# dotnetpower/infomesh

Hardware: AMD Instinct MI355X
Metric: queries/sec (hybrid BM25+dense search, 1.25M docs) (higher is better)
Workload: dtype bf16; 1 GPU; model=bge-small-en(random-init) encoder + BM25 CSR + cosine top-k, global_batch=128, seq_len=32, parallelism=shard1, mode=hybrid, docs_per_gpu=1250000, total_docs=1250000

## Files before the change

### infomesh_amd/index/gpu_index.py

```python
from __future__ import annotations

import math
import re
from dataclasses import dataclass

import numpy as np
import torch

from ..hashing import hash64
from .doc_attrs import (DEAD_BIT, TOP_FETCH, U32_MAX, DocFilter, FacetSpec,
                        TermOps, domain_tables_np, domain_top_np,
                        facet_counts_np, pack_facets, pack_pred,
                        pack_pred_sets, passes, words_i32)

BM25_K1 = 1.2
BM25_B = 0.75
BM25_VOCAB = 1 << 17

MAX_SEGMENTS = 16

COLLAPSE_M_MAX = 4
COLLAPSE_WS_BYTES = 256 << 20


def per_domain_caps(per_domain, B: int) -> list[int] | None:
# ... 80 lines not shown

    def __init__(self, device: str = "cuda", vocab: int = BM25_VOCAB,
                 emb_dtype: str = "bf16"):
        assert emb_dtype in ("bf16", "fp8")
        self.device = torch.device(device)
        self.vocab = vocab
        self.emb_dtype = emb_dtype
        self.n_docs = 0
        self.segments: list[PostingSegment] = []
        self.df: np.ndarray = np.zeros(vocab, dtype=np.int64)
        self._doc_lens = np.zeros(0, dtype=np.int64)
        self.avgdl = 1.0
        self._emb_buf: torch.Tensor | None = None
        self._gid_buf: torch.Tensor | None = None
        self._attr_buf: torch.Tensor | None = None
        self.n_dead = 0
        self._live_bits = None
        self._dom_tables = None
        self._dom_ws: torch.Tensor | None = None
        self._collapse_ws: dict[str, torch.Tensor] = {}
        self._topk = None
        self._topk_dense = None
        self._topk_pruned = None
        self._dense_bmax: dict = {}
        self._dense_graphs: dict = {}
        self.graph_dense = False
        self._h_idf: np.ndarray | None = None
        self._pend_tokens: list[np.ndarray] = []
        self._pend_emb: list[torch.Tensor] = []
        self._pend_gids: list[int] = []
        self._pend_attrs: list = []

    @property
    def embeddings(self) -> torch.Tensor | None:
        if self._emb_buf is None or self.n_docs == 0:
            return None
        return self._emb_buf[:self.n_docs]

    @property
    def global_ids(self) -> torch.Tensor | None:
        if self._gid_buf is None:
            return None
        return self._gid_buf[:self.n_docs]

    @property
    def attrs(self) -> torch.Tensor | None:
        if self._attr_buf is None:
# ... 231 lines not shown
        dl = dl_dev[docs_u.long()].to(torch.int32)
        tfdl = (tf | (dl << 16)).contiguous()
        df_dev = torch.bincount(terms_u, minlength=self.vocab)
        offsets_dev = torch.zeros(self.vocab + 1, dtype=torch.int64,
                                  device=dev)
        torch.cumsum(df_dev, 0, out=offsets_dev[1:])
        df_new = df_dev.cpu().numpy().astype(np.int64)
        seg = PostingSegment(
            offsets=offsets_dev, doc_ids=docs_u.contiguous(),
            tfdl=tfdl, doc_base=self.n_docs, n_docs=n_new,
            h_offs=offsets_dev.cpu().numpy())
        return seg, df_new

    def _upload_t(self, t: torch.Tensor, stream) -> torch.Tensor:
        pinned = t.contiguous().pin_memory()
        with torch.cuda.stream(stream):
            return pinned.to(self.device, non_blocking=True)

    def _invalidate_query_caches(self) -> None:
        self._h_idf = None
        self._dense_graphs = {}
        self._dense_bufs = {}
        self._dense_bmax = {}
        self._bm25_hists = {}
        self._live_bits = None
        self._dom_tables = None
        self._dom_ws = None

    def optimize(self) -> None:
        if len(self.segments) <= 1:
            return
        dev = self.device
        V = self.vocab
        term_parts, doc_parts, tfdl_parts = [], [], []
        arangeV = torch.arange(V, dtype=torch.int64, device=dev)
        for seg in self.segments:
            dfg = seg.offsets.diff()
            term_parts.append(torch.repeat_interleave(arangeV, dfg))
            doc_parts.append(seg.doc_ids.to(torch.int64) + seg.doc_base)
            tfdl_parts.append(seg.tfdl)
        terms = torch.cat(term_parts)
        docs = torch.cat(doc_parts)
        tfdl = torch.cat(tfdl_parts)
        key = terms * self.n_docs + docs
        key, order = torch.sort(key)
        docs_sorted = (key % self.n_docs).to(torch.int32)
# ... 332 lines not shown
        if mark is None:
            def mark(name, t0):
                return t0
        B = len(queries_terms)
        caps = per_domain_caps(per_domain, B)
        dev = self.device
        N = self.n_docs
        k = min(k, N)
        topk = self._get_topk()
        mask = _mask if _mask is not None else self._mask_for(filters, B,
                                                              term_ops)
        tp = _time.perf_counter()
        if scores_buf is not None and scores_buf.shape == (B, N):
            scores = scores_buf
        else:
            scores = torch.empty(B, N, device=dev, dtype=torch.float32)
        qrows, terms = self.dedupe_terms(queries_terms)
        uterms, qt_ut = np.unique(terms, return_inverse=True)
        idf = self._idf_table()[terms]
        qt_off = np.zeros(B + 1, dtype=np.int64)
        np.cumsum(np.bincount(qrows, minlength=B), out=qt_off[1:])
        bd = self._pick_bd(B)
        U = len(uterms)
        hists = getattr(self, "_bm25_hists", None)
        if hists is None:
            hists = self._bm25_hists = {}
        hist = hists.get(B)
        if hist is None:
            hist = hists[B] = torch.zeros(
                B * 256, device=dev, dtype=torch.int32)
        else:
            hist.zero_()
        tp = mark("shard.chunks", tp)
        evt = getattr(self, "_h2d_evt", None)
        if evt is not None:
            evt.synchronize()
        qt_off_d = self._h2d("qt_off", qt_off, torch.int32)
        qt_ut_d = self._h2d("qt_ut", qt_ut, torch.int32)
        qt_idf_d = self._h2d("qt_idf", idf, torch.float32)
        for si, seg in enumerate(self.segments):
            nblocks = (seg.n_docs + bd - 1) // bd
            bounds = self._bounds_ws(U * nblocks * 2)
            K.bm25_block(
                seg.doc_ids, seg.tfdl, qt_off_d, qt_ut_d, qt_idf_d,
                self._h2d(f"qb{si}", seg.h_offs[uterms], torch.int64),
                self._h2d(f"qe{si}", seg.h_offs[uterms + 1], torch.int64),
                bounds, scores, seg.doc_base, seg.n_docs, bd,
                self.avgdl, k1=BM25_K1, b=BM25_B,
                hist1=hist if mask is None else None)
        if dev.type == "cuda":
            if evt is None:
                evt = self._h2d_evt = torch.cuda.Event()
            evt.record()
        tp = mark("shard.bm25", tp)
        counts = None
        if facets is not None:
            rows_t, edges_t, langs_t, desc_t, doms_t = (
                torch.from_numpy(t) for t in facets.tables())
            counts = K.facet_counts(
                scores, rows_t, self.attrs, edges_t, langs_t, desc_t,
                doms_t, **_mask_kw(mask))
            tp = mark("shard.facets", tp)
        dom_top = tally = None
        if facets is not None and facets.top_rows:
            dom_keys, dom_id = self._domain_tables()
            top_rows = torch.tensor(facets.top_rows, dtype=torch.int32)
            D = dom_keys.numel()
            cnt = K.domain_count(
                scores, top_rows, dom_id, D,
                out=self._domain_ws(len(facets.top_rows), D),
                **_mask_kw(mask))
            dom_top = K.domain_select(cnt, dom_keys, TOP_FETCH + 1)
            tally = DomainTally(cnt, dom_keys)
            tp = mark("shard.topdomains", tp)
        if mask is None:
            out = topk(scores, k, ext_hist1=hist)
        else:
            out = topk(scores, k, mask=mask[0], row_pred=mask[1])
        tp = mark("shard.bm25topk", tp)
        if caps is not None:
            self._collapse_rows("bm25", scores, k, caps, mask, out[0],
                                out[1])
            mark("shard.bm25collapse", tp)
        self._bm25_scores_buf = scores
        return out[0], out[1], counts, dom_top, tally

    def search(self, queries_terms: list[np.ndarray],
               query_emb: torch.Tensor | None, k: int = 100,
               scores_buf: torch.Tensor | None = None,
               phase_t: dict | None = None,
               filters: list[DocFilter | None] | None = None,
               term_ops: list[TermOps | None] | None = None,
               facets: FacetSpec | None = None,
               per_domain: list[int | None] | None = None) -> ShardHits:
        import time as _time

        def mark(name, t0):
            if phase_t is None:
# ... 293 lines not shown
```

### infomesh_amd/ops/_ext.py

```python
from __future__ import annotations

import ctypes
from ctypes import c_float, c_int, c_long, c_void_p
from pathlib import Path

from ..errors import GpuExtensionMissing

_LIB: ctypes.CDLL | None = None
_LOAD_ERROR: str | None = None

_SIGNATURES: dict[str, list] = {
    "infomesh_gemm_bf16_nt": [c_void_p, c_void_p, c_void_p, c_void_p,
                              c_int, c_int, c_int, c_int,
                              c_long, c_long, c_long,
                              c_int, c_float, c_int, c_void_p],
    "infomesh_layernorm": [c_void_p, c_void_p, c_void_p, c_void_p,
                           c_void_p, c_void_p, c_long, c_int, c_float,
                           c_long, c_void_p],
    "infomesh_embed_layernorm": [c_void_p, c_void_p, c_void_p, c_void_p,
                                 c_void_p, c_void_p, c_long, c_int, c_int,
                                 c_float, c_void_p],
    "infomesh_rmsnorm": [c_void_p, c_void_p, c_void_p, c_void_p,
                         c_void_p, c_long, c_int, c_float, c_void_p],
    "infomesh_softmax": [c_void_p, c_void_p, c_void_p, c_long, c_int,
# ... 8 lines not shown
    "infomesh_pool": [c_void_p, c_void_p, c_void_p, c_int, c_int, c_int,
                      c_int, c_int, c_void_p],
    "infomesh_argmax": [c_void_p, c_void_p, c_long, c_int, c_void_p],
    "infomesh_topk": [c_void_p, c_void_p, c_void_p, c_void_p, c_int,
                      c_long, c_int, c_void_p, c_void_p],
    "infomesh_topk_masked": [c_void_p, c_void_p, c_void_p, c_void_p, c_int,
                             c_long, c_int, c_void_p, c_void_p, c_long,
                             c_void_p],
    "infomesh_filter_bitmask": [c_void_p, c_void_p, c_void_p, c_long,
                                c_int, c_void_p],
    "infomesh_filter_bitmask_sets": [c_void_p, c_void_p, c_void_p, c_void_p,
                                     c_void_p, c_long, c_int, c_void_p],
    "infomesh_term_bitmask": [c_void_p, c_long, c_void_p, c_void_p,
                              c_void_p, c_void_p, c_int, c_void_p, c_int,
                              c_long, c_long, c_long, c_long, c_void_p],
    "infomesh_term_block_docs": [],
    "infomesh_topk_workspace_u32": [c_int],
    "infomesh_topk_zero_u32": [c_int],
    "infomesh_bm25_block": [c_void_p, c_void_p, c_void_p, c_void_p,
                            c_void_p, c_void_p, c_void_p, c_void_p,
                            c_void_p, c_void_p, c_int, c_int, c_long,
                            c_long, c_long, c_int, c_float, c_float,
                            c_float, c_void_p],
    "infomesh_score_combine": [c_void_p, c_void_p, c_void_p, c_float,
                               c_float, c_long, c_void_p],
    "infomesh_simhash_fingerprint": [c_void_p, c_void_p, c_void_p, c_long,
                                     c_void_p],
    "infomesh_hamming_scan": [c_void_p, c_void_p, c_void_p, c_void_p,
                              c_void_p, c_void_p, c_int, c_long, c_int,
                              c_int, c_void_p],
    "infomesh_attn_decode": [c_void_p, c_void_p, c_void_p, c_void_p,
                             c_void_p, c_int, c_int, c_int, c_int, c_int,
                             c_float, c_void_p],
    "infomesh_attn_decode_split": [c_void_p, c_void_p, c_void_p, c_void_p,
                                   c_void_p, c_void_p, c_int, c_int, c_int,
                                   c_int, c_int, c_int, c_float, c_void_p],
    "infomesh_attn_fused": [c_void_p, c_void_p, c_void_p, c_void_p,
                            c_void_p, c_int, c_int, c_int, c_int, c_int,
                            c_int, c_long, c_long, c_long, c_long, c_long,
                            c_long, c_long, c_long, c_long,
                            c_long, c_long, c_long,
                            c_int, c_float, c_int, c_void_p],
    "infomesh_kv_append": [c_void_p, c_void_p, c_void_p, c_void_p,
                           c_void_p, c_int, c_int, c_int, c_int, c_void_p],
    "infomesh_dense_scores": [c_void_p, c_void_p, c_void_p,
                              c_int, c_long, c_int, c_float, c_void_p],
# ... 5 lines not shown
                               c_long, c_long, c_long,
                               c_int, c_float, c_int, c_void_p],
    "infomesh_gemv_bf16_nt": [c_void_p, c_void_p, c_void_p, c_void_p,
                              c_int, c_int, c_int, c_int,
                              c_long, c_long, c_long,
                              c_int, c_float, c_int, c_void_p],
    "infomesh_qkv_split": [c_void_p, c_void_p, c_void_p, c_void_p,
                           c_void_p, c_void_p, c_void_p,
                           c_int, c_int, c_int, c_int, c_int, c_int,
                           c_void_p],
    "infomesh_merge_heads": [c_void_p, c_void_p, c_int, c_int, c_int,
                             c_int, c_void_p],
    "infomesh_silu_mul_fused": [c_void_p, c_void_p, c_long, c_int,
                                c_void_p],
    "infomesh_gemm_tile": [c_int, c_int, c_int, c_int],
    "infomesh_gemm_bmax_width": [c_int, c_int, c_int, c_int],
    "infomesh_gemm_bf16_nt_bmax": [c_void_p, c_void_p, c_void_p, c_void_p,
                                   c_void_p, c_int, c_int, c_int, c_int,
                                   c_long, c_long, c_long,
                                   c_int, c_float, c_void_p],
    "infomesh_topk_pruned": [c_void_p, c_void_p, c_int, c_void_p, c_void_p,
                             c_void_p, c_int, c_long, c_int, c_void_p],
    "infomesh_topk_pruned_workspace_u32": [c_int, c_long, c_int, c_int],
    "infomesh_topk_pruned_zero_u32": [c_int],
    "infomesh_facet_counts": [c_void_p, c_void_p, c_void_p, c_void_p,
                              c_void_p, c_void_p, c_void_p, c_void_p,
                              c_void_p, c_long, c_void_p, c_int, c_int,
                              c_long, c_long, c_int, c_int, c_int, c_int,
                              c_void_p],
    "infomesh_facet_chunk_docs": [],
    "infomesh_facet_width": [c_int, c_int, c_int],
    "infomesh_facet_slot": [c_int, c_int, c_int],
    "infomesh_domain_count": [c_void_p, c_void_p, c_void_p, c_void_p,
                              c_void_p, c_void_p, c_int, c_int, c_long,
                              c_long, c_int, c_int, c_void_p],
    "infomesh_domain_select": [c_void_p, c_void_p, c_void_p, c_int, c_int,
                               c_int, c_void_p],
    "infomesh_domtop_chunk_docs": [],
    "infomesh_domtop_lds_slots": [],
    "infomesh_domtop_k_max": [],
    "infomesh_domain_best": [c_void_p, c_void_p, c_void_p, c_void_p,
                             c_void_p, c_void_p, c_int, c_int, c_long,
                             c_long, c_int, c_int, c_int, c_int, c_void_p],
    "infomesh_collapse_select": [c_void_p, c_void_p, c_void_p, c_int, c_int,
                                 c_int, c_int, c_void_p],
    "infomesh_collapse_m_max": [],
    "infomesh_collapse_k_max": [],
    "infomesh_collapse_chunk_docs": [],
    "infomesh_collapse_lds_slots": [],
}

_RESTYPES = {"infomesh_topk_workspace_u32": c_long,
             "infomesh_collapse_m_max": c_int,
             "infomesh_collapse_k_max": c_int,
             "infomesh_collapse_chunk_docs": c_int,
             "infomesh_collapse_lds_slots": c_int,
             "infomesh_domtop_chunk_docs": c_int,
             "infomesh_domtop_lds_slots": c_int,
             "infomesh_domtop_k_max": c_int,
             "infomesh_facet_chunk_docs": c_int,
             "infomesh_facet_width": c_int,
             "infomesh_facet_slot": c_int,
             "infomesh_topk_zero_u32": c_long,
             "infomesh_topk_pruned_workspace_u32": c_long,
             "infomesh_topk_pruned_zero_u32": c_long,
             "infomesh_term_block_docs": c_int,
             "infomesh_gemm_bmax_width": c_int,
             "infomesh_gemm_bf16_nt_bmax": c_int,
             "infomesh_dense_scores": c_int,
             "infomesh_dense_scores_fp8": c_int,
             "infomesh_gemm_tile": c_int,
             "infomesh_attn_fused": c_int,
             "infomesh_embed_layernorm": c_int}


def _try_load() -> ctypes.CDLL | None:
    global _LOAD_ERROR
    so = Path(__file__).resolve().parent / "libinfomesh_hip.so"
    if not so.exists():
        _LOAD_ERROR = f"{so} not built"
        return None
    try:
        lib = ctypes.CDLL(str(so))
    except OSError as e:
        _LOAD_ERROR = str(e)
        return None
    for name, argtypes in _SIGNATURES.items():
        fn = getattr(lib, name)
        fn.argtypes = argtypes
        fn.restype = _RESTYPES.get(name)
    import os
    if os.environ.get("INFOMESH_SYNC_DEBUG"):
        return _SyncDebugLib(lib)
    return lib


class _SyncDebugLib:

    def __init__(self, real: ctypes.CDLL):
        self._real = real

    def __getattr__(self, name: str):
        fn = getattr(self._real, name)
        if not name.startswith("infomesh_"):
            return fn

        def checked(*args, _fn=fn, _name=name):
            r = _fn(*args)
            import torch
            if torch.cuda.is_available():
                try:
                    torch.cuda.synchronize()
                except RuntimeError as e:
# ... 27 lines not shown
```

### infomesh_amd/ops/csrc/bm25.hip

```cpp
#include "common.h"

namespace {

DEVINL long lower_bound_i32(const int* __restrict__ a, long lo, long hi,
                            int v) {
  while (lo < hi) {
    const long mid = (lo + hi) >> 1;
    if (a[mid] < v) lo = mid + 1; else hi = mid;
  }
  return lo;
}

__global__ __launch_bounds__(256) void bm25_bounds_kernel(
    const int* __restrict__ doc_ids,
    const long* __restrict__ u_begin,
    const long* __restrict__ u_end,
    int* __restrict__ bounds,
    int U, int nblocks, int BD) {
  const int i = blockIdx.x * blockDim.x + threadIdx.x;
  if (i >= U * nblocks) return;
  const int ut = i / nblocks, blk = i % nblocks;
  const long b = u_begin[ut], e = u_end[ut];
  const long d0 = (long)blk * BD;
  const long lo = lower_bound_i32(doc_ids, b, e, (int)d0);
  const long hi = lower_bound_i32(doc_ids, lo, e, (int)(d0 + BD));
  bounds[2 * i] = (int)(lo - b);
  bounds[2 * i + 1] = (int)(hi - b);
}

template <bool HIST>
__global__ __launch_bounds__(256) void bm25_block_kernel(
    const int* __restrict__ doc_ids,
    const unsigned int* __restrict__ tfdl,
    const int* __restrict__ qt_off,
    const int* __restrict__ qt_ut,
    const float* __restrict__ qt_idf,
    const long* __restrict__ u_begin,
    const int* __restrict__ bounds,
    float* __restrict__ scores,
    unsigned* __restrict__ hist1,
    long rowN, long doc_base, long nseg, int BD, int nblocks,
    float norm_a, float norm_b, float k1p1) {
  extern __shared__ float lds_scores[];
  const int q = blockIdx.x;
  const int blk = blockIdx.y;
  const long d0 = (long)blk * BD;
  const int nd = (int)min((long)BD, nseg - d0);
  unsigned* lh = reinterpret_cast<unsigned*>(lds_scores + BD);
  for (int i = threadIdx.x; i < nd; i += blockDim.x) lds_scores[i] = 0.0f;
  if (HIST) hist8_zero(lh);
  __syncthreads();
  const int t0 = qt_off[q], t1 = qt_off[q + 1];
  for (int ti = t0; ti < t1; ++ti) {
    const int ut = qt_ut[ti];
    const int* bp = bounds + 2 * ((long)ut * nblocks + blk);
    const long base = u_begin[ut];
    const long lo = base + bp[0], hi = base + bp[1];
    const float w = qt_idf[ti] * k1p1;
    for (long p = lo + threadIdx.x; p < hi; p += blockDim.x) {
      const int d = doc_ids[p] - (int)d0;
      const unsigned int td = tfdl[p];
      const float tf = (float)(td & 0xffffu);
      const float dl = (float)(td >> 16);
      atomicAdd(&lds_scores[d], w * tf / (tf + norm_a + norm_b * dl));
    }
    __syncthreads();
  }
  float* __restrict__ srow = scores + (long)q * rowN + doc_base + d0;
  if (!HIST) {
    for (int i = threadIdx.x; i < nd; i += blockDim.x)
      __builtin_nontemporal_store(lds_scores[i], srow + i);
    return;
  }
  unsigned* my = hist8_mine(lh);
  unsigned zc = 0;
  for (int i = threadIdx.x; i < nd; i += blockDim.x) {
    const float v = lds_scores[i];
    __builtin_nontemporal_store(v, srow + i);
    if (v == 0.0f) ++zc;
    else atomicAdd(&my[float_to_ordered(v) >> 24], 1u);
  }
  for (int off = WAVE / 2; off; off >>= 1)
    zc += __shfl_xor(zc, off, WAVE);
  constexpr unsigned ZBIN = 0x80000000u >> 24;
  if ((threadIdx.x % WAVE) == 0 && zc)
    atomicAdd(&my[ZBIN], zc);
  __syncthreads();
  hist8_merge(lh, hist1 + (long)q * 256);
}

__global__ void combine_kernel(const float* __restrict__ a,
                               const float* __restrict__ b,
                               float* __restrict__ out,
                               float wa, float wb, long n) {
  const long idx = (long)blockIdx.x * blockDim.x + threadIdx.x;
  for (long i = idx; i < n; i += (long)gridDim.x * blockDim.x)
    out[i] = wa * a[i] + wb * b[i];
}

}

extern "C" void infomesh_bm25_block(
    const void* doc_ids, const void* tfdl, const void* qt_off,
    const void* qt_ut, const void* qt_idf, const void* u_begin,
    const void* u_end, void* bounds, void* scores, void* hist1,
    int B, int U, long rowN, long doc_base, long nseg,
    int BD, float norm_a, float norm_b, float k1p1, void* stream) {
  if (nseg <= 0 || B <= 0) return;
  auto s = reinterpret_cast<hipStream_t>(stream);
  const int nblocks = (int)((nseg + BD - 1) / BD);
  if (U > 0) {
    const int total = U * nblocks;
    hipLaunchKernelGGL(bm25_bounds_kernel,
                       dim3((unsigned)((total + 255) / 256)), dim3(256), 0, s,
                       (const int*)doc_ids, (const long*)u_begin,
                       (const long*)u_end, (int*)bounds, U, nblocks, BD);
  }
  dim3 grid((unsigned)B, (unsigned)nblocks);
  const size_t shm = (size_t)BD * sizeof(float)
      + (hist1 ? HIST8_U32 * sizeof(unsigned) : 0);
  if (hist1)
    hipLaunchKernelGGL(bm25_block_kernel<true>, grid, dim3(256), shm, s,
                       (const int*)doc_ids, (const unsigned int*)tfdl,
                       (const int*)qt_off, (const int*)qt_ut,
                       (const float*)qt_idf, (const long*)u_begin,
                       (const int*)bounds, (float*)scores,
                       (unsigned*)hist1,
                       rowN, doc_base, nseg, BD, nblocks,
                       norm_a, norm_b, k1p1);
  else
    hipLaunchKernelGGL(bm25_block_kernel<false>, grid, dim3(256), shm, s,
                       (const int*)doc_ids, (const unsigned int*)tfdl,
                       (const int*)qt_off, (const int*)qt_ut,
                       (const float*)qt_idf, (const long*)u_begin,
                       (const int*)bounds, (float*)scores, nullptr,
                       rowN, doc_base, nseg, BD, nblocks,
                       norm_a, norm_b, k1p1);
}

extern "C" void infomesh_score_combine(const void* a, const void* b,
                                       void* out, float wa, float wb,
                                       long n, void* stream) {
  auto s = reinterpret_cast<hipStream_t>(stream);
  long blocks = min((n + 255) / 256, (long)2048);
  hipLaunchKernelGGL(combine_kernel, dim3((unsigned)blocks), dim3(256), 0, s,
                     (const float*)a, (const float*)b, (float*)out, wa, wb, n);
}
```

### infomesh_amd/ops/csrc/topk.hip

```cpp
#include "common.h"

#define TOPK_CAP 8192

#define HI_RES 4096

namespace {

struct MaskRef {
  const unsigned* bits;
  const int* row_pred;
  long W;
};
DEVINL const unsigned* mask_row(const MaskRef& m, int b) {
  return m.bits + (long)m.row_pred[b] * m.W;
}
DEVINL unsigned mask_nibble(const unsigned* __restrict__ mrow, long i) {
  return (mrow[i >> 3] >> ((unsigned)(i & 7) * 4)) & 15u;
}
DEVINL void keep_loaded(float4& v) {
  asm volatile("" : "+v"(v.x), "+v"(v.y), "+v"(v.z), "+v"(v.w));
}
DEVINL bool mask_bit(const unsigned* __restrict__ mrow, long col) {
  return (mrow[col >> 5] >> (unsigned)(col & 31)) & 1u;
}
// ... 254 lines not shown
      const unsigned long long v = d[i];
      out_vals[(long)b * K + i] = ordered_to_float(~(unsigned)(v >> 32));
      out_idx[(long)b * K + i] = (int)(v & 0xffffffffu);
    } else {
      out_vals[(long)b * K + i] = -INFINITY;
      out_idx[(long)b * K + i] = -1;
    }
  }
}

struct TopkLayout {
  long hist1, hist2, bin1, chi1, thresh, shift, cnt, cnt_eq, cand, total;
  explicit TopkLayout(long B)
      : hist1(0), hist2(hist1 + B * 256), bin1(hist2 + B * 256),
        chi1(bin1 + B), thresh(chi1 + B), shift(thresh + B),
        cnt(shift + B), cnt_eq(cnt + B),
        cand((cnt_eq + B + 1) & ~1L),
        total(cand + B * TOPK_CAP * 2) {}
};
unsigned long long* cand_of(unsigned* ws, long B) {
  return reinterpret_cast<unsigned long long*>(ws + TopkLayout(B).cand);
}

#define PRUNE_THREADS 1024
#define PRUNE_PAD 0xffffffffu
__global__ __launch_bounds__(PRUNE_THREADS) void gather_blocks_kernel(
    const float* __restrict__ scores, const int* __restrict__ ids,
    int* __restrict__ blk, float* __restrict__ gath, long N, long NB,
    int W, int K1) {
  __shared__ int d[1024];
  const int b = blockIdx.x;
  int n2 = 64;
  while (n2 < K1) n2 <<= 1;
  for (int i = threadIdx.x; i < n2; i += blockDim.x)
    d[i] = i < K1 ? ids[(long)b * K1 + i] : 0x7fffffff;
  __syncthreads();
  for (int k = 2; k <= n2; k <<= 1) {
    for (int j = k >> 1; j > 0; j >>= 1) {
      for (int i = threadIdx.x; i < n2; i += blockDim.x) {
        const int ixj = i ^ j;
        if (ixj > i) {
          const bool up = ((i & k) == 0);
          const int a = d[i], c = d[ixj];
          if ((a > c) == up) { d[i] = c; d[ixj] = a; }
        }
      }
      __syncthreads();
    }
  }
  for (int i = threadIdx.x; i < K1; i += blockDim.x)
    blk[(long)b * K1 + i] = d[i];
  const float* row = scores + (long)b * N;
  float* grow = gath + (long)b * K1 * W;
  for (int e = threadIdx.x; e < K1 * W; e += blockDim.x) {
    const long id = d[e / W];
    const long col = id * W + e % W;
    grow[e] = (id >= 0 && id < NB && col < N) ? row[col]
                                              : __uint_as_float(PRUNE_PAD);
  }
}

__global__ __launch_bounds__(256) void remap_blocks_kernel(
    const int* __restrict__ blk, float* __restrict__ out_vals,
    int* __restrict__ out_idx, long N, int W, int K1, int K) {
  const int b = blockIdx.x;
  for (int i = threadIdx.x; i < K; i += blockDim.x) {
    const int p = out_idx[(long)b * K + i];
    if (p < 0) continue;
    const long col = (long)blk[(long)b * K1 + p / W] * W + p % W;
    if (col < N) {
      out_idx[(long)b * K + i] = (int)col;
    } else {
      out_vals[(long)b * K + i] = -INFINITY;
      out_idx[(long)b * K + i] = -1;
    }
  }
}

struct PrunedLayout {
  long K1, zero2, cand, vals1, idx1, blk, gath, total;
  PrunedLayout(long B, long NB, long K, long W)
      : K1(K < NB ? K : NB), zero2(TopkLayout(B).cand), cand(2 * zero2),
        vals1(cand + B * TOPK_CAP * 2), idx1(vals1 + B * K1),
        blk(idx1 + B * K1),
        gath((blk + B * K1 + 3) & ~3L),
        total(gath + B * K1 * W) {}
};

}

extern "C" long infomesh_topk_workspace_u32(int B) {
  return TopkLayout(B).total;
}

extern "C" long infomesh_topk_zero_u32(int B) { return TopkLayout(B).cand; }

template <bool MASKED, typename... M>
static void topk_launch(const void* scores, unsigned* ws,
                        unsigned long long* cand, void* out_vals,
                        void* out_idx, int B, long N, int K,
                        const void* ext_hist1, hipStream_t s, M... mask) {
  static_assert(sizeof...(M) == (MASKED ? 1 : 0), "one MaskRef iff MASKED");
  const TopkLayout L(B);

  int chunks = (int)min((N + 256 * 64 - 1) / (256 * 64), (long)1024);
  if (chunks < 1) chunks = 1;
  dim3 g1(chunks, B), blk(256);
  const unsigned* h1 = (const unsigned*)ext_hist1;
  if (!h1) {
    h1 = ws + L.hist1;
// ... 17 lines not shown
                     (int*)out_idx, K);
}

extern "C" void infomesh_topk(const void* scores, void* workspace,
                              void* out_vals, void* out_idx,
                              int B, long N, int K,
                              const void* ext_hist1, void* stream) {
  unsigned* ws = reinterpret_cast<unsigned*>(workspace);
  topk_launch<false>(scores, ws, cand_of(ws, B), out_vals, out_idx, B, N, K,
                     ext_hist1, reinterpret_cast<hipStream_t>(stream));
}

extern "C" void infomesh_topk_masked(const void* scores, void* workspace,
                                     void* out_vals, void* out_idx,
                                     int B, long N, int K,
                                     const void* bits, const void* row_pred,
                                     long W, void* stream) {
  unsigned* ws = reinterpret_cast<unsigned*>(workspace);
  topk_launch<true>(scores, ws, cand_of(ws, B), out_vals, out_idx, B, N, K,
                    nullptr, reinterpret_cast<hipStream_t>(stream),
                    MaskRef{(const unsigned*)bits, (const int*)row_pred, W});
}

extern "C" long infomesh_topk_pruned_workspace_u32(int B, long N, int K,
                                                   int W) {
  return PrunedLayout(B, (N + W - 1) / W, K, W).total;
}
extern "C" long infomesh_topk_pruned_zero_u32(int B) {
  return 2 * TopkLayout(B).cand;
}

extern "C" void infomesh_topk_pruned(const void* scores, const void* bmax,
                                     int W, void* workspace, void* out_vals,
                                     void* out_idx, int B, long N, int K,
                                     void* stream) {
  hipStream_t s = reinterpret_cast<hipStream_t>(stream);
  unsigned* ws = reinterpret_cast<unsigned*>(workspace);
  const long NB = (N + W - 1) / W;
  const PrunedLayout L(B, NB, K, W);
  const int K1 = (int)L.K1;
  auto* cand = reinterpret_cast<unsigned long long*>(ws + L.cand);
  int* idx1 = reinterpret_cast<int*>(ws + L.idx1);
  int* blk = reinterpret_cast<int*>(ws + L.blk);
  float* gath = reinterpret_cast<float*>(ws + L.gath);
  topk_launch<false>(bmax, ws, cand, ws + L.vals1, idx1, B, NB, K1, nullptr,
                     s);
  hipLaunchKernelGGL(gather_blocks_kernel, dim3(B), dim3(PRUNE_THREADS), 0,
                     s, (const float*)scores, idx1, blk, gath, N, NB, W, K1);
  topk_launch<false>(gath, ws + L.zero2, cand, out_vals, out_idx, B,
                     (long)K1 * W, K, nullptr, s);
  hipLaunchKernelGGL(remap_blocks_kernel, dim3(B), dim3(256), 0, s, blk,
                     (float*)out_vals, (int*)out_idx, N, W, K1, K);
}
```

### infomesh_amd/ops/kernels.py

```python
from __future__ import annotations

import torch

from . import _ext

ACT = {"none": 0, "gelu": 1, "silu": 2, "relu": 3, "tanh": 4}


def _ptr(t: torch.Tensor | None) -> int | None:
    return None if t is None else t.data_ptr()


def _check(t: torch.Tensor, dtype: torch.dtype, name: str) -> None:
    assert t.is_cuda, f"{name} must be on GPU"
    assert t.dtype == dtype, f"{name} must be {dtype}, got {t.dtype}"
    assert t.is_contiguous(), f"{name} must be contiguous"


def gemm_route(M: int, N: int, K: int, G: int) -> str:
    if M <= 16:
        return "gemv"
    if (M >= 4096 and N >= 512 and K % 64 == 0
            and ((M + 255) // 256) * ((N + 255) // 256) * max(G, 1) >= 224):
        return "gemm8"
# ... 312 lines not shown
                scores.data_ptr(), self._ws.data_ptr(), vals.data_ptr(),
                idx.data_ptr(), B, N, k, mask.data_ptr(),
                row_pred.data_ptr(), mask.shape[1], _ext.stream_ptr())
            return vals, idx
        lib.infomesh_topk(scores.data_ptr(), self._ws.data_ptr(),
                          vals.data_ptr(), idx.data_ptr(), B, N, k,
                          0 if ext_hist1 is None else ext_hist1.data_ptr(),
                          _ext.stream_ptr())
        return vals, idx


class TopKPruned:

    def __init__(self, device: torch.device | str = "cuda"):
        self.device = torch.device(device)
        self._ws: torch.Tensor | None = None

    def __call__(self, scores: torch.Tensor, bmax: torch.Tensor, W: int,
                 k: int) -> tuple[torch.Tensor, torch.Tensor]:
        assert scores.dim() == 2
        _check(scores, torch.float32, "scores")
        _check(bmax, torch.float32, "bmax")
        B, N = scores.shape
        assert 1 <= k <= 1024 and W > 0
        assert bmax.shape == (B, (N + W - 1) // W), \
            f"bmax must be [B, ceil(N/W)], got {tuple(bmax.shape)}"
        lib = _ext.lib()
        nu32 = lib.infomesh_topk_pruned_workspace_u32(B, N, k, W)
        if self._ws is None or self._ws.numel() < nu32:
            self._ws = torch.empty(nu32, device=scores.device,
                                   dtype=torch.int32)
        self._ws[:lib.infomesh_topk_pruned_zero_u32(B)].zero_()
        vals = torch.empty((B, k), device=scores.device, dtype=torch.float32)
        idx = torch.empty((B, k), device=scores.device, dtype=torch.int32)
        lib.infomesh_topk_pruned(
            scores.data_ptr(), bmax.data_ptr(), W, self._ws.data_ptr(),
            vals.data_ptr(), idx.data_ptr(), B, N, k, _ext.stream_ptr())
        return vals, idx


def topk(scores: torch.Tensor, k: int) -> tuple[torch.Tensor, torch.Tensor]:
    return TopK(scores.device)(scores, k)


def filter_bitmask(attrs: torch.Tensor, preds: torch.Tensor) -> torch.Tensor:
    _check(attrs, torch.int32, "attrs")
    _check(preds, torch.int32, "preds")
    assert attrs.dim() == 2 and attrs.shape[1] == 4
    assert preds.dim() == 2 and preds.shape[1] == 4 and preds.shape[0] >= 1
    N, P = attrs.shape[0], preds.shape[0]
    assert P <= 65535
    W = (N + 63) // 64 * 2
    bits = torch.empty((P, W), device=attrs.device, dtype=torch.int32)
    _ext.lib().infomesh_filter_bitmask(
        attrs.data_ptr(), preds.data_ptr(), bits.data_ptr(), N, P,
        _ext.stream_ptr())
    return bits


FILTER_SETS_MAX = 2048
# ... 331 lines not shown
    m, R, D = best.shape
    if not 1 <= m <= collapse_m_max():
        raise ValueError(
            f"collapse_select: m = {m}; 1 <= m <= {collapse_m_max()}")
    if not 1 <= k <= collapse_k_max():
        raise ValueError(
            f"collapse_select: k = {k}; 1 <= k <= {collapse_k_max()}")
    assert R >= 1 and D >= 1, "best: [m, R, D]"
    vals = torch.empty((R, k), device=best.device, dtype=torch.float32)
    idx = torch.empty((R, k), device=best.device, dtype=torch.int32)
    _ext.lib().infomesh_collapse_select(
        best.data_ptr(), vals.data_ptr(), idx.data_ptr(), R, D, m, k,
        _ext.stream_ptr())
    return vals, idx


def bm25_block(doc_ids: torch.Tensor, tfdl: torch.Tensor,
               qt_off: torch.Tensor, qt_ut: torch.Tensor,
               qt_idf: torch.Tensor, u_begin: torch.Tensor,
               u_end: torch.Tensor, bounds: torch.Tensor,
               scores: torch.Tensor, doc_base: int, nseg: int,
               bd: int, avgdl: float, k1: float = 1.2,
               b: float = 0.75,
               hist1: torch.Tensor | None = None) -> torch.Tensor:
    B, N = scores.shape
    U = u_begin.numel()
    nblocks = (nseg + bd - 1) // bd
    _check(scores, torch.float32, "scores")
    assert nblocks <= 65535 and qt_off.numel() == B + 1
    assert doc_ids.dtype == torch.int32 and tfdl.dtype == torch.int32
    assert bounds.numel() >= U * nblocks * 2
    assert bd * 4 + (8448 if hist1 is not None else 0) <= 160 * 1024
    if hist1 is not None:
        assert hist1.dtype == torch.int32 and hist1.numel() >= B * 256
    norm_a = k1 * (1.0 - b)
    norm_b = k1 * b / max(avgdl, 1e-9)
    _ext.lib().infomesh_bm25_block(
        doc_ids.data_ptr(), tfdl.data_ptr(), qt_off.data_ptr(),
        qt_ut.data_ptr(), qt_idf.data_ptr(), u_begin.data_ptr(),
        u_end.data_ptr(), bounds.data_ptr(), scores.data_ptr(),
        0 if hist1 is None else hist1.data_ptr(),
        B, U, N, doc_base, nseg, bd,
        norm_a, norm_b, k1 + 1.0, _ext.stream_ptr())
    return scores


def score_combine(a: torch.Tensor, b: torch.Tensor, wa: float,
                  wb: float) -> torch.Tensor:
    out = torch.empty_like(a)
    _ext.lib().infomesh_score_combine(a.data_ptr(), b.data_ptr(),
                                      out.data_ptr(), wa, wb, a.numel(),
                                      _ext.stream_ptr())
    return out


def simhash_fingerprint(offsets: torch.Tensor,
                        hashes: torch.Tensor) -> torch.Tensor:
    ndocs = offsets.numel() - 1
    out = torch.empty(ndocs, device=offsets.device, dtype=torch.int64)
    _ext.lib().infomesh_simhash_fingerprint(
        offsets.data_ptr(), hashes.data_ptr(), out.data_ptr(), ndocs,
        _ext.stream_ptr())
    return out

# ... 129 lines not shown
```

Before: 44570 queries/s.

## Emit per-64-doc block maxima from BM25 and use single-kernel pruned top-k

The BM25 scoring kernel gains a variant that writes, alongside the scores, the maximum score of every 64-document block. The BM25 top-k then goes through a rewritten pruned selector: a row-parallel radix select over block maxima picks candidate blocks, and only those blocks' scores are scanned. This replaces the old multi-launch pruned pipeline (two top-k passes, gather, remap) and the histogram path. The new path is on by default when no filter mask is present, at the cost of an extra bmax buffer and more complex kernels.

```diff
diff --git a/infomesh_amd/index/gpu_index.py b/infomesh_amd/index/gpu_index.py
--- a/infomesh_amd/index/gpu_index.py
+++ b/infomesh_amd/index/gpu_index.py
@@ -1,6 +1,7 @@
 from __future__ import annotations
 
 import math
+import os
 import re
 from dataclasses import dataclass
 
@@ -127,7 +128,10 @@
         self._topk = None
         self._topk_dense = None
         self._topk_pruned = None
+        self._topk_pruned_bm25 = None
         self._dense_bmax: dict = {}
+        self.bm25_pruned = os.environ.get("INFOMESH_BM25_PRUNED") != "0"
+        self._bm25_bmax: dict = {}
         self._dense_graphs: dict = {}
         self.graph_dense = False
         self._h_idf: np.ndarray | None = None
@@ -405,6 +409,7 @@
         self._dense_graphs = {}
         self._dense_bufs = {}
         self._dense_bmax = {}
+        self._bm25_bmax = {}
         self._bm25_hists = {}
         self._live_bits = None
         self._dom_tables = None
@@ -783,15 +788,24 @@
         np.cumsum(np.bincount(qrows, minlength=B), out=qt_off[1:])
         bd = self._pick_bd(B)
         U = len(uterms)
-        hists = getattr(self, "_bm25_hists", None)
-        if hists is None:
-            hists = self._bm25_hists = {}
-        hist = hists.get(B)
-        if hist is None:
-            hist = hists[B] = torch.zeros(
-                B * 256, device=dev, dtype=torch.int32)
-        else:
-            hist.zero_()
+        pruned = (mask is None and self.bm25_pruned and dev.type == "cuda"
+                  and all(s.doc_base % 64 == 0 for s in self.segments))
+        bmax = hist = None
+        if pruned:
+            bmax = self._bm25_bmax.get(B)
+            if bmax is None or bmax.shape != (B, (N + 63) // 64):
+                bmax = self._bm25_bmax[B] = torch.empty(
+                    B, (N + 63) // 64, device=dev, dtype=torch.float32)
+        elif mask is None:
+            hists = getattr(self, "_bm25_hists", None)
+            if hists is None:
+                hists = self._bm25_hists = {}
+            hist = hists.get(B)
+            if hist is None:
+                hist = hists[B] = torch.zeros(
+                    B * 256, device=dev, dtype=torch.int32)
+            else:
+                hist.zero_()
         tp = mark("shard.chunks", tp)
         evt = getattr(self, "_h2d_evt", None)
         if evt is not None:
@@ -808,7 +822,7 @@
                 self._h2d(f"qe{si}", seg.h_offs[uterms + 1], torch.int64),
                 bounds, scores, seg.doc_base, seg.n_docs, bd,
                 self.avgdl, k1=BM25_K1, b=BM25_B,
-                hist1=hist if mask is None else None)
+                hist1=hist, bmax=bmax)
         if dev.type == "cuda":
             if evt is None:
                 evt = self._h2d_evt = torch.cuda.Event()
@@ -834,7 +848,11 @@
             dom_top = K.domain_select(cnt, dom_keys, TOP_FETCH + 1)
             tally = DomainTally(cnt, dom_keys)
             tp = mark("shard.topdomains", tp)
-        if mask is None:
+        if pruned:
+            if self._topk_pruned_bm25 is None:
+                self._topk_pruned_bm25 = K.TopKPruned(dev)
+            out = self._topk_pruned_bm25(scores, bmax, 64, k)
+        elif mask is None:
             out = topk(scores, k, ext_hist1=hist)
         else:
             out = topk(scores, k, mask=mask[0], row_pred=mask[1])
diff --git a/infomesh_amd/ops/_ext.py b/infomesh_amd/ops/_ext.py
--- a/infomesh_amd/ops/_ext.py
+++ b/infomesh_amd/ops/_ext.py
@@ -54,6 +54,11 @@
                             c_void_p, c_void_p, c_int, c_int, c_long,
                             c_long, c_long, c_int, c_float, c_float,
                             c_float, c_void_p],
+    "infomesh_bm25_block_bmax": [c_void_p, c_void_p, c_void_p, c_void_p,
+                                 c_void_p, c_void_p, c_void_p, c_void_p,
+                                 c_void_p, c_void_p, c_int, c_int, c_long,
+                                 c_long, c_long, c_int, c_float, c_float,
+                                 c_float, c_void_p],
     "infomesh_score_combine": [c_void_p, c_void_p, c_void_p, c_float,
                                c_float, c_long, c_void_p],
     "infomesh_simhash_fingerprint": [c_void_p, c_void_p, c_void_p, c_long,
@@ -105,7 +110,6 @@
     "infomesh_topk_pruned": [c_void_p, c_void_p, c_int, c_void_p, c_void_p,
                              c_void_p, c_int, c_long, c_int, c_void_p],
     "infomesh_topk_pruned_workspace_u32": [c_int, c_long, c_int, c_int],
-    "infomesh_topk_pruned_zero_u32": [c_int],
     "infomesh_facet_counts": [c_void_p, c_void_p, c_void_p, c_void_p,
                               c_void_p, c_void_p, c_void_p, c_void_p,
                               c_void_p, c_long, c_void_p, c_int, c_int,
@@ -145,8 +149,8 @@
              "infomesh_facet_width": c_int,
              "infomesh_facet_slot": c_int,
              "infomesh_topk_zero_u32": c_long,
+             "infomesh_topk_pruned": c_int,
              "infomesh_topk_pruned_workspace_u32": c_long,
-             "infomesh_topk_pruned_zero_u32": c_long,
              "infomesh_term_block_docs": c_int,
              "infomesh_gemm_bmax_width": c_int,
              "infomesh_gemm_bf16_nt_bmax": c_int,
@@ -157,6 +161,17 @@
              "infomesh_embed_layernorm": c_int}
 
 
+def bind(so: Path | str, strict: bool = True) -> ctypes.CDLL:
+    lib = ctypes.CDLL(str(so))
+    for name, argtypes in _SIGNATURES.items():
+        if not strict and not hasattr(lib, name):
+            continue
+        fn = getattr(lib, name)
+        fn.argtypes = argtypes
+        fn.restype = _RESTYPES.get(name)
+    return lib
+
+
 def _try_load() -> ctypes.CDLL | None:
     global _LOAD_ERROR
     so = Path(__file__).resolve().parent / "libinfomesh_hip.so"
@@ -164,14 +179,10 @@
         _LOAD_ERROR = f"{so} not built"
         return None
     try:
-        lib = ctypes.CDLL(str(so))
+        lib = bind(so)
     except OSError as e:
         _LOAD_ERROR = str(e)
         return None
-    for name, argtypes in _SIGNATURES.items():
-        fn = getattr(lib, name)
-        fn.argtypes = argtypes
-        fn.restype = _RESTYPES.get(name)
     import os
     if os.environ.get("INFOMESH_SYNC_DEBUG"):
         return _SyncDebugLib(lib)
diff --git a/infomesh_amd/ops/csrc/bm25.hip b/infomesh_amd/ops/csrc/bm25.hip
--- a/infomesh_amd/ops/csrc/bm25.hip
+++ b/infomesh_amd/ops/csrc/bm25.hip
@@ -1,4 +1,5 @@
 #include "common.h"
+#include "gemm_common.h"
 
 namespace {
 
@@ -28,7 +29,7 @@
   bounds[2 * i + 1] = (int)(hi - b);
 }
 
-template <bool HIST>
+template <bool HIST, bool BMAX = false>
 __global__ __launch_bounds__(256) void bm25_block_kernel(
     const int* __restrict__ doc_ids,
     const unsigned int* __restrict__ tfdl,
@@ -39,6 +40,7 @@
     const int* __restrict__ bounds,
     float* __restrict__ scores,
     unsigned* __restrict__ hist1,
+    float* __restrict__ bmax,
     long rowN, long doc_base, long nseg, int BD, int nblocks,
     float norm_a, float norm_b, float k1p1) {
   extern __shared__ float lds_scores[];
@@ -67,6 +69,28 @@
     __syncthreads();
   }
   float* __restrict__ srow = scores + (long)q * rowN + doc_base + d0;
+  if (BMAX) {
+    float* __restrict__ brow =
+        bmax + (long)q * ((rowN + WAVE - 1) / WAVE) + (doc_base + d0) / WAVE;
+    const int lane = threadIdx.x % WAVE;
+    for (int base = 0; base < nd; base += blockDim.x) {
+      const int i = base + threadIdx.x;
+      unsigned bits = 0;
+      if (i < nd) {
+        const float v = lds_scores[i];
+        __builtin_nontemporal_store(v, srow + i);
+        bits = __float_as_uint(v);
+      }
+      bits = group_max_u32<16>(bits);
+      const unsigned m = max(
+          max((unsigned)__builtin_amdgcn_readlane((int)bits, 0),
+              (unsigned)__builtin_amdgcn_readlane((int)bits, 16)),
+          max((unsigned)__builtin_amdgcn_readlane((int)bits, 32),
+              (unsigned)__builtin_amdgcn_readlane((int)bits, 48)));
+      if (lane == 0 && i < nd) brow[i / WAVE] = __uint_as_float(m);
+    }
+    return;
+  }
   if (!HIST) {
     for (int i = threadIdx.x; i < nd; i += blockDim.x)
       __builtin_nontemporal_store(lds_scores[i], srow + i);
@@ -100,11 +124,11 @@
 
 }
 
-extern "C" void infomesh_bm25_block(
+static void bm25_launch(
     const void* doc_ids, const void* tfdl, const void* qt_off,
     const void* qt_ut, const void* qt_idf, const void* u_begin,
     const void* u_end, void* bounds, void* scores, void* hist1,
-    int B, int U, long rowN, long doc_base, long nseg,
+    void* bmax, int B, int U, long rowN, long doc_base, long nseg,
     int BD, float norm_a, float norm_b, float k1p1, void* stream) {
   if (nseg <= 0 || B <= 0) return;
   auto s = reinterpret_cast<hipStream_t>(stream);
@@ -119,13 +143,22 @@
   dim3 grid((unsigned)B, (unsigned)nblocks);
   const size_t shm = (size_t)BD * sizeof(float)
       + (hist1 ? HIST8_U32 * sizeof(unsigned) : 0);
-  if (hist1)
+  if (bmax)
+    hipLaunchKernelGGL((bm25_block_kernel<false, true>), grid, dim3(256),
+                       (size_t)BD * sizeof(float), s,
+                       (const int*)doc_ids, (const unsigned int*)tfdl,
+                       (const int*)qt_off, (const int*)qt_ut,
+                       (const float*)qt_idf, (const long*)u_begin,
+                       (const int*)bounds, (float*)scores, nullptr,
+                       (float*)bmax, rowN, doc_base, nseg, BD, nblocks,
+                       norm_a, norm_b, k1p1);
+  else if (hist1)
     hipLaunchKernelGGL(bm25_block_kernel<true>, grid, dim3(256), shm, s,
                        (const int*)doc_ids, (const unsigned int*)tfdl,
                        (const int*)qt_off, (const int*)qt_ut,
                        (const float*)qt_idf, (const long*)u_begin,
                        (const int*)bounds, (float*)scores,
-                       (unsigned*)hist1,
+                       (unsigned*)hist1, nullptr,
                        rowN, doc_base, nseg, BD, nblocks,
                        norm_a, norm_b, k1p1);
   else
@@ -133,9 +166,31 @@
                        (const int*)doc_ids, (const unsigned int*)tfdl,
                        (const int*)qt_off, (const int*)qt_ut,
                        (const float*)qt_idf, (const long*)u_begin,
-                       (const int*)bounds, (float*)scores, nullptr,
+                       (const int*)bounds, (float*)scores, nullptr, nullptr,
                        rowN, doc_base, nseg, BD, nblocks,
                        norm_a, norm_b, k1p1);
+}
+
+extern "C" void infomesh_bm25_block(
+    const void* doc_ids, const void* tfdl, const void* qt_off,
+    const void* qt_ut, const void* qt_idf, const void* u_begin,
+    const void* u_end, void* bounds, void* scores, void* hist1,
+    int B, int U, long rowN, long doc_base, long nseg,
+    int BD, float norm_a, float norm_b, float k1p1, void* stream) {
+  bm25_launch(doc_ids, tfdl, qt_off, qt_ut, qt_idf, u_begin, u_end, bounds,
+              scores, hist1, nullptr, B, U, rowN, doc_base, nseg, BD, norm_a,
+              norm_b, k1p1, stream);
+}
+
+extern "C" void infomesh_bm25_block_bmax(
+    const void* doc_ids, const void* tfdl, const void* qt_off,
+    const void* qt_ut, const void* qt_idf, const void* u_begin,
+    const void* u_end, void* bounds, void* scores, void* bmax,
+    int B, int U, long rowN, long doc_base, long nseg,
+    int BD, float norm_a, float norm_b, float k1p1, void* stream) {
+  bm25_launch(doc_ids, tfdl, qt_off, qt_ut, qt_idf, u_begin, u_end, bounds,
+              scores, nullptr, bmax, B, U, rowN, doc_base, nseg, BD, norm_a,
+              norm_b, k1p1, stream);
 }
 
 extern "C" void infomesh_score_combine(const void* a, const void* b,
diff --git a/infomesh_amd/ops/csrc/topk.hip b/infomesh_amd/ops/csrc/topk.hip
--- a/infomesh_amd/ops/csrc/topk.hip
+++ b/infomesh_amd/ops/csrc/topk.hip
@@ -300,70 +300,262 @@
   return reinterpret_cast<unsigned long long*>(ws + TopkLayout(B).cand);
 }
 
-#define PRUNE_THREADS 1024
-#define PRUNE_PAD 0xffffffffu
-__global__ __launch_bounds__(PRUNE_THREADS) void gather_blocks_kernel(
-    const float* __restrict__ scores, const int* __restrict__ ids,
-    int* __restrict__ blk, float* __restrict__ gath, long N, long NB,
-    int W, int K1) {
-  __shared__ int d[1024];
+#define ROW_THREADS 1024
+#define ROW_WAVES (ROW_THREADS / WAVE)
+#define ROW_STAGE 24576
+#define ROW_U_LDS 4
+#define ROW_U_MEM 16
+#define ROW_GROUP_MAX (ROW_STAGE / 1024)
+
+DEVINL unsigned row_key(float f) {
+  const unsigned o = float_to_ordered(f);
+  return o == 0x7fffffffu ? 0x80000000u : o;
+}
+
+struct RowLds {
+  unsigned stage[ROW_STAGE];
+  unsigned hist[HIST8_U32];
+  unsigned bins[256];
+  unsigned wave_gt[ROW_WAVES], wave_eq[ROW_WAVES];
+  unsigned sel_bin, sel_cum;
+  int blk[1024];
+  int grp[1024];
+  unsigned long long sort[1024];
+};
+
+DEVINL unsigned lane_rank(unsigned long long m) {
+  return __builtin_amdgcn_mbcnt_hi((unsigned)(m >> 32),
+                                   __builtin_amdgcn_mbcnt_lo((unsigned)m, 0));
+}
+
+template <int U, typename KeyAt>
+DEVINL unsigned row_radix_select(RowLds& l, long n, unsigned K,
+                                 unsigned& above, KeyAt key_at) {
+  const int lane = threadIdx.x & (WAVE - 1);
+  unsigned prefix = 0, cum = 0;
+  for (int sh = 24; sh >= 0; sh -= 8) {
+    hist8_zero(l.hist);
+    __syncthreads();
+    unsigned* my = hist8_mine(l.hist);
+    for (long base = threadIdx.x; base < n; base += ROW_THREADS * U) {
+      unsigned o[U];
+#pragma unroll
+      for (int u = 0; u < U; ++u) {
+        const long i = base + (long)u * ROW_THREADS;
+        o[u] = i < n ? key_at(i) : 0u;
+      }
+#pragma unroll
+      for (int u = 0; u < U; ++u) {
+        if (base + (long)u * ROW_THREADS < n &&
+            (sh == 24 || (o[u] >> sh >> 8) == prefix))
+          atomicAdd(&my[(o[u] >> sh) & 255], 1u);
+      }
+    }
+    __syncthreads();
+    if (threadIdx.x < 256) {
+      unsigned sum = 0;
+#pragma unroll
+      for (int c = 0; c < HIST8_COPIES; ++c)
+        sum += l.hist[c * HIST8_STRIDE + threadIdx.x];
+      l.bins[threadIdx.x] = sum;
+    }
+    __syncthreads();
+    if (threadIdx.x < WAVE) {
+      unsigned c[4], tot = 0;
+#pragma unroll
+      for (int j = 0; j < 4; ++j) {
+        c[j] = l.bins[255 - 4 * lane - j];
+        tot += c[j];
+      }
+      unsigned inc = tot;
+#pragma unroll
+      for (int off = 1; off < WAVE; off <<= 1) {
+        const unsigned v = __shfl_up(inc, off, WAVE);
+        if (lane >= off) inc += v;
+      }
+      unsigned run = cum + inc - tot;
+      int hit = -1;
+#pragma unroll
+      for (int j = 0; j < 4; ++j) {
+        if (hit < 0) {
+          if (run + c[j] >= K) hit = j; else run += c[j];
+        }
+      }
+      const unsigned long long found = __ballot(hit >= 0);
+      if (found == 0) {
+        if (lane == WAVE - 1) { l.sel_bin = 0; l.sel_cum = run - c[3]; }
+      } else if (lane == __ffsll((long long)found) - 1) {
+        l.sel_bin = 255 - 4 * lane - hit;
+        l.sel_cum = run;
+      }
+    }
+    __syncthreads();
+    prefix = (prefix << 8) | l.sel_bin;
+    cum = l.sel_cum;
+  }
+  above = cum;
+  return prefix;
+}
+
+template <int U, typename KeyAt, typename Take>
+DEVINL void row_ordered_take(RowLds& l, long n, unsigned t, unsigned need_eq,
+                             KeyAt key_at, Take take) {
+  const int lane = threadIdx.x & (WAVE - 1), w = threadIdx.x / WAVE;
+  const long per =
+      ((n + ROW_WAVES - 1) / ROW_WAVES + WAVE - 1) & ~(long)(WAVE - 1);
+  const long lo = min(w * per, n), hi = min(lo + per, n);
+  unsigned ng = 0, ne = 0;
+  for (long base = lo; base < hi; base += WAVE * U) {
+    unsigned o[U];
+#pragma unroll
+    for (int u = 0; u < U; ++u) {
+      const long i = base + u * WAVE + lane;
+      o[u] = i < hi ? key_at(i) : 0u;
+    }
+#pragma unroll
+    for (int u = 0; u < U; ++u) {
+      const bool in = base + u * WAVE + lane < hi;
+      ng += __popcll(__ballot(in && o[u] > t));
+      ne += __popcll(__ballot(in && o[u] == t));
+    }
+  }
+  if (lane == 0) { l.wave_gt[w] = ng; l.wave_eq[w] = ne; }
+  __syncthreads();
+  unsigned og = 0, oe = 0;
+  for (int v = 0; v < w; ++v) { og += l.wave_gt[v]; oe += l.wave_eq[v]; }
+  for (long base = lo; base < hi; base += WAVE * U) {
+    unsigned o[U];
+#pragma unroll
+    for (int u = 0; u < U; ++u) {
+      const long i = base + u * WAVE + lane;
+      o[u] = i < hi ? key_at(i) : 0u;
+    }
+#pragma unroll
+    for (int u = 0; u < U; ++u) {
+      const long i = base + u * WAVE + lane;
+      const bool gt = i < hi && o[u] > t, eq = i < hi && o[u] == t;
+      const unsigned long long mg = __ballot(gt), me = __ballot(eq);
+      const unsigned rg = og + lane_rank(mg), re = oe + lane_rank(me);
+      if (gt || (eq && re < need_eq)) take(i, o[u], rg + min(re, need_eq));
+      og += __popcll(mg);
+      oe += __popcll(me);
+    }
+  }
+  __syncthreads();
+}
+
+__global__ __launch_bounds__(256) void group_max_kernel(
+    const float* __restrict__ bmax, float* __restrict__ gmax, long NB,
+    long NG, int G) {
+  const long j = (long)blockIdx.x * blockDim.x + threadIdx.x;
+  if (j >= NG) return;
+  const float* __restrict__ mrow = bmax + (long)blockIdx.y * NB;
+  unsigned m = 0;
+  for (long i = j * G; i < min(j * G + G, NB); ++i)
+    m = max(m, row_key(mrow[i]));
+  gmax[(long)blockIdx.y * NG + j] = ordered_to_float(m);
+}
+
+__global__ __launch_bounds__(ROW_THREADS) void row_select_kernel(
+    const float* __restrict__ scores, const float* __restrict__ bmax,
+    const float* __restrict__ gmax, float* __restrict__ out_vals,
+    int* __restrict__ out_idx, long N, long NB, long NG, unsigned G,
+    unsigned W, int K1, int K) {
+  __shared__ RowLds l;
   const int b = blockIdx.x;
-  int n2 = 64;
-  while (n2 < K1) n2 <<= 1;
-  for (int i = threadIdx.x; i < n2; i += blockDim.x)
-    d[i] = i < K1 ? ids[(long)b * K1 + i] : 0x7fffffff;
-  __syncthreads();
-  for (int k = 2; k <= n2; k <<= 1) {
+  const float* __restrict__ mrow = bmax + (long)b * NB;
+  const float* __restrict__ row = scores + (long)b * N;
+
+  for (int i = threadIdx.x; i < 1024; i += ROW_THREADS) l.blk[i] = 0;
+  unsigned above, t;
+  auto take_block = [&](long i, unsigned, unsigned pos) {
+    if (pos < (unsigned)K1) l.blk[pos] = (int)i;
+  };
+  auto key_at = [&](long i) { return l.stage[i]; };
+  if (G == 1) {
+    for (long i = threadIdx.x; i < NB; i += ROW_THREADS)
+      l.stage[i] = row_key(mrow[i]);
+    t = row_radix_select<ROW_U_LDS>(l, NB, (unsigned)K1, above, key_at);
+    row_ordered_take<ROW_U_LDS>(l, NB, t, (unsigned)K1 - above, key_at,
+                                take_block);
+  } else {
+    const float* __restrict__ grow = gmax + (long)b * NG;
+    const unsigned KG = (unsigned)min((long)K1, NG);
+    for (int i = threadIdx.x; i < 1024; i += ROW_THREADS) l.grp[i] = 0;
+    for (long i = threadIdx.x; i < NG; i += ROW_THREADS)
+      l.stage[i] = row_key(grow[i]);
+    t = row_radix_select<ROW_U_LDS>(l, NG, KG, above, key_at);
+    row_ordered_take<ROW_U_LDS>(
+        l, NG, t, KG - above, key_at, [&](long i, unsigned, unsigned pos) {
+          if (pos < KG) l.grp[pos] = (int)i;
+        });
+    const unsigned n1 = KG * G;
+    auto blk_of = [&](unsigned e) { return (long)l.grp[e / G] * G + e % G; };
+    for (unsigned e = threadIdx.x; e < n1; e += ROW_THREADS) {
+      const long id = blk_of(e);
+      l.stage[e] = id < NB ? row_key(mrow[id]) : 0u;
+    }
+    t = row_radix_select<ROW_U_LDS>(l, n1, (unsigned)K1, above, key_at);
+    row_ordered_take<ROW_U_LDS>(
+        l, n1, t, (unsigned)K1 - above, key_at,
+        [&](long e, unsigned, unsigned pos) {
+          const long id = blk_of((unsigned)e);
+          if (pos < (unsigned)K1 && id < NB) l.blk[pos] = (int)id;
+        });
+  }
+
+  const unsigned n2 = (unsigned)K1 * W;
+  auto col_of = [&](unsigned e) { return (long)l.blk[e / W] * W + e % W; };
+  auto take_score = [&](long e, unsigned o, unsigned pos) {
+    const long col = col_of((unsigned)e);
+    if (pos < (unsigned)K && col < N)
+      l.sort[pos] = ((unsigned long long)(~o) << 32) | (unsigned)col;
+  };
+  for (int i = threadIdx.x; i < 1024; i += ROW_THREADS) l.sort[i] = ~0ULL;
+  unsigned T;
+  if (n2 <= ROW_STAGE) {
+    for (unsigned e = threadIdx.x; e < n2; e += ROW_THREADS) {
+      const long col = col_of(e);
+      l.stage[e] = col < N ? row_key(row[col]) : 0u;
+    }
+    T = row_radix_select<ROW_U_LDS>(l, n2, (unsigned)K, above, key_at);
+    row_ordered_take<ROW_U_LDS>(l, n2, T, (unsigned)K - above, key_at,
+                                take_score);
+  } else {
+    auto mem_key_at = [&](long e) {
+      const long col = col_of((unsigned)e);
+      return col < N ? row_key(row[col]) : 0u;
+    };
+    T = row_radix_select<ROW_U_MEM>(l, n2, (unsigned)K, above, mem_key_at);
+    row_ordered_take<ROW_U_MEM>(l, n2, T, (unsigned)K - above, mem_key_at,
+                                take_score);
+  }
+
+  int ns = 64;
+  while (ns < K) ns <<= 1;
+  for (int k = 2; k <= ns; k <<= 1) {
     for (int j = k >> 1; j > 0; j >>= 1) {
-      for (int i = threadIdx.x; i < n2; i += blockDim.x) {
-        const int ixj = i ^ j;
-        if (ixj > i) {
-          const bool up = ((i & k) == 0);
-          const int a = d[i], c = d[ixj];
-          if ((a > c) == up) { d[i] = c; d[ixj] = a; }
-        }
+      const int i = threadIdx.x, ixj = i ^ j;
+      if (i < ns && ixj > i) {
+        const bool up = ((i & k) == 0);
+        const unsigned long long a = l.sort[i], c = l.sort[ixj];
+        if ((a > c) == up) { l.sort[i] = c; l.sort[ixj] = a; }
       }
       __syncthreads();
     }
   }
-  for (int i = threadIdx.x; i < K1; i += blockDim.x)
-    blk[(long)b * K1 + i] = d[i];
-  const float* row = scores + (long)b * N;
-  float* grow = gath + (long)b * K1 * W;
-  for (int e = threadIdx.x; e < K1 * W; e += blockDim.x) {
-    const long id = d[e / W];
-    const long col = id * W + e % W;
-    grow[e] = (id >= 0 && id < NB && col < N) ? row[col]
-                                              : __uint_as_float(PRUNE_PAD);
-  }
-}
-
-__global__ __launch_bounds__(256) void remap_blocks_kernel(
-    const int* __restrict__ blk, float* __restrict__ out_vals,
-    int* __restrict__ out_idx, long N, int W, int K1, int K) {
-  const int b = blockIdx.x;
-  for (int i = threadIdx.x; i < K; i += blockDim.x) {
-    const int p = out_idx[(long)b * K + i];
-    if (p < 0) continue;
-    const long col = (long)blk[(long)b * K1 + p / W] * W + p % W;
-    if (col < N) {
-      out_idx[(long)b * K + i] = (int)col;
-    } else {
-      out_vals[(long)b * K + i] = -INFINITY;
-      out_idx[(long)b * K + i] = -1;
-    }
-  }
-}
-
-struct PrunedLayout {
-  long K1, zero2, cand, vals1, idx1, blk, gath, total;
-  PrunedLayout(long B, long NB, long K, long W)
-      : K1(K < NB ? K : NB), zero2(TopkLayout(B).cand), cand(2 * zero2),
-        vals1(cand + B * TOPK_CAP * 2), idx1(vals1 + B * K1),
-        blk(idx1 + B * K1),
-        gath((blk + B * K1 + 3) & ~3L),
-        total(gath + B * K1 * W) {}
-};
+  for (int i = threadIdx.x; i < K; i += ROW_THREADS) {
+    const unsigned long long v = l.sort[i];
+    const bool real = v != ~0ULL;
+    out_vals[(long)b * K + i] =
+        real ? ordered_to_float(~(unsigned)(v >> 32)) : -INFINITY;
+    out_idx[(long)b * K + i] = real ? (int)(v & 0xffffffffu) : -1;
+  }
+}
+
+long row_group(long NB) {
+  return NB <= ROW_STAGE ? 1 : (NB + ROW_STAGE - 1) / ROW_STAGE;
+}
 
 }
 
@@ -427,33 +619,29 @@
                     MaskRef{(const unsigned*)bits, (const int*)row_pred, W});
 }
 
+extern "C" int infomesh_topk_pruned(const void* scores, const void* bmax,
+                                    int W, void* workspace, void* out_vals,
+                                    void* out_idx, int B, long N, int K,
+                                    void* stream) {
+  if (B <= 0) return 0;
+  hipStream_t s = reinterpret_cast<hipStream_t>(stream);
+  const long NB = (N + W - 1) / W;
+  const int K1 = (int)(K < NB ? K : NB);
+  const long G = row_group(NB), NG = (NB + G - 1) / G;
+  if (G > ROW_GROUP_MAX) return 1;
+  if (G > 1)
+    hipLaunchKernelGGL(group_max_kernel, dim3((unsigned)((NG + 255) / 256), B),
+                       dim3(256), 0, s, (const float*)bmax, (float*)workspace,
+                       NB, NG, (int)G);
+  hipLaunchKernelGGL(row_select_kernel, dim3(B), dim3(ROW_THREADS), 0, s,
+                     (const float*)scores, (const float*)bmax,
+                     (const float*)workspace, (float*)out_vals, (int*)out_idx,
+                     N, NB, NG, (unsigned)G, (unsigned)W, K1, K);
+  return 0;
+}
+
 extern "C" long infomesh_topk_pruned_workspace_u32(int B, long N, int K,
                                                    int W) {
-  return PrunedLayout(B, (N + W - 1) / W, K, W).total;
-}
-extern "C" long infomesh_topk_pruned_zero_u32(int B) {
-  return 2 * TopkLayout(B).cand;
-}
-
-extern "C" void infomesh_topk_pruned(const void* scores, const void* bmax,
-                                     int W, void* workspace, void* out_vals,
-                                     void* out_idx, int B, long N, int K,
-                                     void* stream) {
-  hipStream_t s = reinterpret_cast<hipStream_t>(stream);
-  unsigned* ws = reinterpret_cast<unsigned*>(workspace);
-  const long NB = (N + W - 1) / W;
-  const PrunedLayout L(B, NB, K, W);
-  const int K1 = (int)L.K1;
-  auto* cand = reinterpret_cast<unsigned long long*>(ws + L.cand);
-  int* idx1 = reinterpret_cast<int*>(ws + L.idx1);
-  int* blk = reinterpret_cast<int*>(ws + L.blk);
-  float* gath = reinterpret_cast<float*>(ws + L.gath);
-  topk_launch<false>(bmax, ws, cand, ws + L.vals1, idx1, B, NB, K1, nullptr,
-                     s);
-  hipLaunchKernelGGL(gather_blocks_kernel, dim3(B), dim3(PRUNE_THREADS), 0,
-                     s, (const float*)scores, idx1, blk, gath, N, NB, W, K1);
-  topk_launch<false>(gath, ws + L.zero2, cand, out_vals, out_idx, B,
-                     (long)K1 * W, K, nullptr, s);
-  hipLaunchKernelGGL(remap_blocks_kernel, dim3(B), dim3(256), 0, s, blk,
-                     (float*)out_vals, (int*)out_idx, N, W, K1, K);
-}
+  const long NB = (N + W - 1) / W, G = row_group(NB);
+  return G > 1 ? (long)B * ((NB + G - 1) / G) : 0;
+}
diff --git a/infomesh_amd/ops/kernels.py b/infomesh_amd/ops/kernels.py
--- a/infomesh_amd/ops/kernels.py
+++ b/infomesh_amd/ops/kernels.py
@@ -358,20 +358,21 @@
         _check(scores, torch.float32, "scores")
         _check(bmax, torch.float32, "bmax")
         B, N = scores.shape
-        assert 1 <= k <= 1024 and W > 0
+        assert 1 <= k <= 1024 and 0 < W <= 1 << 20
         assert bmax.shape == (B, (N + W - 1) // W), \
             f"bmax must be [B, ceil(N/W)], got {tuple(bmax.shape)}"
+        vals = torch.empty((B, k), device=scores.device, dtype=torch.float32)
+        idx = torch.empty((B, k), device=scores.device, dtype=torch.int32)
         lib = _ext.lib()
         nu32 = lib.infomesh_topk_pruned_workspace_u32(B, N, k, W)
-        if self._ws is None or self._ws.numel() < nu32:
+        if nu32 and (self._ws is None or self._ws.numel() < nu32):
             self._ws = torch.empty(nu32, device=scores.device,
                                    dtype=torch.int32)
-        self._ws[:lib.infomesh_topk_pruned_zero_u32(B)].zero_()
-        vals = torch.empty((B, k), device=scores.device, dtype=torch.float32)
-        idx = torch.empty((B, k), device=scores.device, dtype=torch.int32)
-        lib.infomesh_topk_pruned(
-            scores.data_ptr(), bmax.data_ptr(), W, self._ws.data_ptr(),
+        rc = lib.infomesh_topk_pruned(
+            scores.data_ptr(), bmax.data_ptr(), W,
+            self._ws.data_ptr() if nu32 else 0,
             vals.data_ptr(), idx.data_ptr(), B, N, k, _ext.stream_ptr())
+        assert rc == 0, f"topk_pruned: {N} columns at W = {W} is too wide"
         return vals, idx
 
 
@@ -749,7 +750,8 @@
                scores: torch.Tensor, doc_base: int, nseg: int,
                bd: int, avgdl: float, k1: float = 1.2,
                b: float = 0.75,
-               hist1: torch.Tensor | None = None) -> torch.Tensor:
+               hist1: torch.Tensor | None = None,
+               bmax: torch.Tensor | None = None) -> torch.Tensor:
     B, N = scores.shape
     U = u_begin.numel()
     nblocks = (nseg + bd - 1) // bd
@@ -760,13 +762,25 @@
     assert bd * 4 + (8448 if hist1 is not None else 0) <= 160 * 1024
     if hist1 is not None:
         assert hist1.dtype == torch.int32 and hist1.numel() >= B * 256
+    if bmax is not None:
+        assert hist1 is None, "bmax and hist1 are mutually exclusive"
+        _check(bmax, torch.float32, "bmax")
+        assert bmax.shape == (B, (N + 63) // 64), \
+            f"bmax must be [B, ceil(N/64)], got {tuple(bmax.shape)}"
+        assert doc_base % 64 == 0 and bd % 64 == 0, \
+            "bmax: segment base and doc-block must be multiples of 64"
     norm_a = k1 * (1.0 - b)
     norm_b = k1 * b / max(avgdl, 1e-9)
-    _ext.lib().infomesh_bm25_block(
+    lib = _ext.lib()
+    if bmax is not None:
+        fn, side = lib.infomesh_bm25_block_bmax, bmax.data_ptr()
+    else:
+        fn = lib.infomesh_bm25_block
+        side = 0 if hist1 is None else hist1.data_ptr()
+    fn(
         doc_ids.data_ptr(), tfdl.data_ptr(), qt_off.data_ptr(),
         qt_ut.data_ptr(), qt_idf.data_ptr(), u_begin.data_ptr(),
-        u_end.data_ptr(), bounds.data_ptr(), scores.data_ptr(),
-        0 if hist1 is None else hist1.data_ptr(),
+        u_end.data_ptr(), bounds.data_ptr(), scores.data_ptr(), side,
         B, U, N, doc_base, nseg, bd,
         norm_a, norm_b, k1 + 1.0, _ext.stream_ptr())
     return scores
```

Result: faster. 50400 queries/s (median of 6 runs) (+13.1%).
